# stjude-rust-labs/ngs

Measured on AMD Instinct MI355X. Metric: BAM records/sec (whole node), all qc facets, 150 bp reads, higher is better.
Workload: dtype u8/u32 integer (u64 accumulators)

## Files before the change

ngs_amd/csrc/qual_kernel.hip:

```cpp
#include <hip/hip_runtime.h>

#include <cstdlib>

#include "kernels.h"

namespace ngsq {

typedef unsigned long long u64;

__host__ __device__ constexpr uint32_t qw_rp(uint32_t R) {
    const uint32_t want = R < 12 ? R : 12;
    for (uint32_t rp = R; rp < R + 8; rp++) {
        const uint32_t s = (4 * rp) % 32, d = s < 32 - s ? s : 32 - s;
        if (d >= want) return rp;
    }
    return R;
}
__host__ __device__ constexpr uint32_t qw_cp(uint32_t R) { return (16 * qw_rp(R) + 31) / 32 * 32; }

uint32_t qual_window_lds_bytes(uint32_t R) { return QUAL_BINS * qw_cp(R) * 4; }

template <uint32_t R>
__global__ __launch_bounds__(1024) void k_qual_win(DeviceState st, const uint8_t *__restrict__ qual, uint64_t n_rec,
                                                   uint32_t pitch) {
    NGSQ_FOREGROUND_WAVE();
    constexpr uint32_t RP = qw_rp(R), CP = qw_cp(R), CP4 = CP * 4, RP4 = RP * 4;
    constexpr uint32_t S4 = 4u * RP4;
    constexpr uint32_t magicR = R == 1 ? 0u : (uint32_t)(((1ull << 32) + R - 1) / R);
    extern __shared__ uint32_t s_q[];
    constexpr uint32_t nb = QUAL_BINS * CP;
    for (uint32_t i = threadIdx.x; i < nb; i += blockDim.x) s_q[i] = 0;
    __syncthreads();

    const uint32_t rem = pitch - 16u * (R - 1);
    const uint64_t n_win = n_rec * R;
    const uint64_t per = (n_win + gridDim.x - 1) / gridDim.x;
    const uint64_t lo = min(per * blockIdx.x, n_win), hi = min(lo + per, n_win);
    const uint64_t rec_lo = lo / R;
    const uint32_t tl0 = (uint32_t)(lo - rec_lo * R) + threadIdx.x;
    const uint32_t rl0 = R == 1 ? tl0 : __umulhi(tl0, magicR);
    uint32_t w = tl0 - rl0 * R;
    uint32_t rot = rl0 & 3u;
    constexpr uint32_t STEP_R = 1024 / R, STEP_W = 1024 % R;
    const uint32_t d0 = STEP_R * pitch + 16u * STEP_W, d1 = d0 + pitch - 16u * R;
    const uint8_t *p = qual + (rec_lo + rl0) * (uint64_t)pitch + 16u * w;
    uint32_t bad = 0;
    char *const tab = reinterpret_cast<char *>(s_q);

    auto exact = [&](const uint32_t (&x)[4], uint32_t w_) {
        const uint32_t nvalid = (w_ == R - 1) ? rem : 16u;
        for (uint32_t j = 0; j < nvalid; j++) {
            const uint32_t q = (x[j >> 2] >> (8 * (j & 3))) & 0xFFu;
            if (q <= NGSQ_MAX_SCORE)
                atomicAdd(reinterpret_cast<uint32_t *>(tab + q * CP4 + 4u * w_ + j * RP4), 1u);
            else if (q != 0xFFu)
                bad += 1;
        }
    };
    auto tally = [&](const uint4 &cur, uint32_t w_, uint32_t rot_) {
        const uint32_t ww[4] = {cur.x, cur.y, cur.z, cur.w};
        const uint32_t any = (ww[0] | ww[1] | ww[2] | ww[3]) & 0xC0C0C0C0u;
        if (__builtin_expect(any == 0u, 1)) {
            const uint32_t wbase = 4u * w_;
            uint32_t x[4], bd[4];
            const bool r1 = rot_ & 1u, r2 = rot_ & 2u;
            const uint32_t y0 = r2 ? ww[2] : ww[0], y1 = r2 ? ww[3] : ww[1], y2 = r2 ? ww[0] : ww[2],
                           y3 = r2 ? ww[1] : ww[3];
            x[0] = r1 ? y1 : y0;
            x[1] = r1 ? y0 : y1;
            x[2] = r1 ? y3 : y2;
            x[3] = r1 ? y2 : y3;
            const uint32_t h = r2 ? 2u * S4 : 0u, l = r1 ? S4 : 0u;
            bd[0] = wbase + h + l;
            bd[1] = wbase + h + (S4 - l);
            bd[2] = wbase + (2u * S4 - h) + l;
            bd[3] = wbase + (2u * S4 - h) + (S4 - l);
#pragma unroll
            for (uint32_t d = 0; d < 4; d++) {
#pragma unroll
                for (uint32_t k = 0; k < 4; k++) {
                    const uint32_t q = (x[d] >> (8 * k)) & 0xFFu;
                    atomicAdd(reinterpret_cast<uint32_t *>(tab + (__umul24(q, CP4) + bd[d]) + k * RP4), 1u);
                }
            }
        } else {
            exact(ww, w_);
        }
    };
    auto load = [&](const uint8_t *q) -> uint4 {
        uint4 v;
        __builtin_memcpy(&v, q, 16);
        return v;
    };

    const uint64_t hi_fast = min(hi, n_win - 1);
    uint64_t t = lo + threadIdx.x;
    if (t < hi_fast) {
        uint4 cur = load(p);
        while (t + 1024 < hi_fast) {
            uint32_t w_n = w + STEP_W;
            const bool wrap = w_n >= R;
            w_n = wrap ? w_n - R : w_n;
            p += wrap ? d1 : d0;
            const uint4 nxt = load(p);
            tally(cur, w, rot);
            cur = nxt;
            w = w_n;
            rot = (rot + STEP_R + (wrap ? 1u : 0u)) & 3u;
            t += 1024;
        }
        tally(cur, w, rot);
        t += 1024;
    }
    if (hi == n_win && n_win > 0 && (n_win - 1 - lo) % 1024 == threadIdx.x && n_win - 1 >= lo) {
        uint32_t x[4] = {0, 0, 0, 0};
        const uint64_t off = (n_rec - 1) * (uint64_t)pitch + 16u * (R - 1);
        for (uint32_t k = 0; k < rem; k++) x[k >> 2] |= (uint32_t)qual[off + k] << (8 * (k & 3));
        exact(x, R - 1);
    }
    __syncthreads();
    const uint32_t n_out = pitch * QUAL_BINS;
    for (uint32_t i = threadIdx.x; i < n_out; i += blockDim.x) {
        const uint32_t c = i / QUAL_BINS, q = i - c * QUAL_BINS;
        const uint32_t v = s_q[q * CP + (c & 15u) * RP + (c >> 4)];
        if (v) atomicAdd(&st.counters[st.off_qual + i], (u64)v);
    }
    uint32_t r = bad;
#pragma unroll
    for (int o = 32; o > 0; o >>= 1) r += __shfl_down(r, o, 64);
    if ((threadIdx.x & 63) == 0 && r) atomicAdd(&st.counters[C_ERR + E_BAD_QUAL], (u64)r);
}

__device__ __forceinline__ uint32_t qr_wave_inclusive_sum(uint32_t v) {
    v += (uint32_t)__builtin_amdgcn_update_dpp(0, (int)v, 0x111, 0xF, 0xF, false);
    v += (uint32_t)__builtin_amdgcn_update_dpp(0, (int)v, 0x112, 0xF, 0xF, false);
    v += (uint32_t)__builtin_amdgcn_update_dpp(0, (int)v, 0x114, 0xF, 0xF, false);
    v += (uint32_t)__builtin_amdgcn_update_dpp(0, (int)v, 0x118, 0xF, 0xF, false);
    v += (uint32_t)__builtin_amdgcn_update_dpp(0, (int)v, 0x142, 0xA, 0xF, false);
    v += (uint32_t)__builtin_amdgcn_update_dpp(0, (int)v, 0x143, 0xC, 0xF, false);
    return v;
}
constexpr uint32_t QR_ROWS = 64;
constexpr uint32_t QR_TRASH = QR_ROWS;
constexpr uint32_t QR_FLUSH_EVERY = 63;
__host__ __device__ constexpr uint32_t qr_cp(uint32_t R) { return (8 * qw_rp(R) + 31) / 32 * 32; }
__host__ __device__ constexpr uint32_t qr_table_bytes(uint32_t R) { return (QR_ROWS + 1) * qr_cp(R) * 4; }
__device__ __forceinline__ uint32_t qr_from_lane(uint32_t v, uint32_t src_lane) {
    return (uint32_t)__builtin_amdgcn_ds_bpermute((int)(src_lane << 2), (int)v);
}

template <uint32_t R>
__global__ __launch_bounds__(1024) void k_qual_ragged(DeviceState st, const uint8_t *__restrict__ qual,
                                                      const uint64_t *__restrict__ qual_off, uint64_t n_rec) {
    NGSQ_FOREGROUND_WAVE();
    constexpr uint32_t RP = qw_rp(R), CP = qr_cp(R), CP4 = CP * 4, RP4 = RP * 4;
    constexpr uint32_t S4 = 2u * RP4;
    extern __shared__ uint32_t s_q[];
    constexpr uint32_t nb = (QR_ROWS + 1) * CP;
    for (uint32_t i = threadIdx.x; i < nb; i += blockDim.x) s_q[i] = 0;
    char *const tab = reinterpret_cast<char *>(s_q);
    const uint32_t lane = threadIdx.x & 63u, wave = threadIdx.x >> 6;
    uint8_t *const map = reinterpret_cast<uint8_t *>(s_q + nb) + wave * (64u * R);
    uint4 *const keep_tab = reinterpret_cast<uint4 *>(reinterpret_cast<uint8_t *>(s_q + nb) + 16u * 64u * R);
    if (threadIdx.x <= 16u) {
        uint32_t k[4];
        for (uint32_t d = 0; d < 4; d++) {
            const uint32_t nvd = threadIdx.x > 4u * d ? min(threadIdx.x - 4u * d, 4u) : 0u;
            k[d] = nvd >= 4u ? 0xFFFFFFFFu : (1u << (8u * nvd)) - 1u;
        }
        keep_tab[threadIdx.x] = make_uint4(k[0], k[1], k[2], k[3]);
    }
    __syncthreads();
    const uint64_t per = (n_rec + gridDim.x - 1) / gridDim.x;
    const uint64_t lo = min(per * blockIdx.x, n_rec), hi = min(lo + per, n_rec);
    const uint64_t end_bytes = n_rec ? qual_off[n_rec] : 0;
    uint32_t bad = 0, too_long = 0;
    u64 *const gq = st.counters + st.off_qual;
    const uint32_t n_cyc = min(st.max_read_len, 16u * R);
    auto flush = [&]() {
        __syncthreads();
        for (uint32_t i = threadIdx.x; i < n_cyc * QR_ROWS; i += blockDim.x) {
            const uint32_t c = i / QR_ROWS, q = i - c * QR_ROWS, kb = c & 15u;
            const uint32_t v = (s_q[q * CP + (kb >> 1) * RP + (c >> 4)] >> (16u * (kb & 1u))) & 0xFFFFu;
            if (v) atomicAdd(&gq[(uint64_t)c * QUAL_BINS + q], (u64)v);
        }
        __syncthreads();
        for (uint32_t i = threadIdx.x; i < QR_ROWS * CP; i += blockDim.x) s_q[i] = 0;
        __syncthreads();
    };

    auto load_offs = [&](uint64_t i0, uint64_t &o0, uint64_t &o1) {
        const uint64_t rec = i0 + lane;
        o0 = qual_off[rec < n_rec ? rec : n_rec];
        o1 = qual_off[rec + 1 < n_rec ? rec + 1 : n_rec];
    };
    uint64_t nx_o0 = 0, nx_o1 = 0;
    if (lo + 64ull * wave < hi) load_offs(lo + 64ull * wave, nx_o0, nx_o1);
    const uint64_t n_iter = (hi - lo + 1023) / 1024;
    for (uint64_t it = 0; it < n_iter; it++) {
        if (it && it % QR_FLUSH_EVERY == 0) flush();
        const uint64_t i0 = lo + it * 1024 + 64ull * wave;
        if (i0 >= hi) continue;
        const uint64_t rec = i0 + lane;
        const uint64_t cur_o0 = nx_o0, cur_o1 = nx_o1;
        load_offs(i0 + 64ull * 16, nx_o0, nx_o1);
        uint64_t off = 0;
        uint32_t len = 0;
        if (rec < hi) {
            off = cur_o0;
            const uint64_t l64 = cur_o1 - off;
            len = (uint32_t)min(l64, (uint64_t)st.max_read_len);
            too_long += l64 > st.max_read_len;
        }
        const uint32_t nwin = (len + 15u) >> 4;
        const uint32_t P = qr_wave_inclusive_sum(nwin);
        const uint32_t T = __builtin_amdgcn_readlane(P, 63);
        const uint64_t off0 = ((uint64_t)(uint32_t)__builtin_amdgcn_readfirstlane((int)(off >> 32)) << 32) |
                              (uint32_t)__builtin_amdgcn_readfirstlane((int)(uint32_t)off);
        const uint32_t rel = rec < hi ? (uint32_t)(off - off0) : 0u;
        const uint32_t first_win = P - nwin;
        const uint32_t fw_len = first_win | len << 16;
        for (uint32_t j = 0; __ballot(j < nwin); j++)
            if (j < nwin) map[first_win + j] = (uint8_t)lane;
        __builtin_amdgcn_fence(__ATOMIC_ACQ_REL, "wavefront");
        __builtin_amdgcn_wave_barrier();
        struct Sched {
            uint32_t r, w, nv, sh;
            bool active;
            uint4 v;
        };
        const uint64_t g0 = min(off0, end_bytes - 16);
        const uint32_t delta = (uint32_t)(off0 - g0), lim = (uint32_t)min(end_bytes - 16 - g0, (uint64_t)0xFFFFFFFFu);
        const uint8_t *const gbase = qual + g0;
        auto fetch = [&](uint32_t t0) -> Sched {
            Sched sc;
            const uint32_t t = t0 + lane;
            sc.active = t < T;
            const uint32_t tt = sc.active ? t : (t0 < T ? t0 : 0u);
            sc.r = map[tt];
            const uint32_t fl = qr_from_lane(fw_len, sc.r);
            sc.w = tt - (fl & 0xFFFFu);
            const uint32_t l = fl >> 16;
            sc.nv = sc.w == (l >> 4) ? (l & 15u) : 16u;
            const uint32_t at = qr_from_lane(rel, sc.r) + 16u * sc.w + delta, at_c = min(at, lim);
            sc.sh = at - at_c;
            __builtin_memcpy(&sc.v, gbase + at_c, 16);
            return sc;
        };
        Sched nx{};
        if (T) nx = fetch(0);
        for (uint32_t t0 = 0; t0 < T; t0 += 64) {
            const Sched cu = nx;
            nx = fetch(t0 + 64 < T ? t0 + 64 : t0);
            const bool active = cu.active;
            const uint32_t r = cu.r, w = cu.w, nv = cu.nv;
            if (!active) continue;
            uint32_t ww[4] = {cu.v.x, cu.v.y, cu.v.z, cu.v.w};
            if (__builtin_expect(cu.sh != 0u, 0)) {
                u64 l64 = (u64)ww[1] << 32 | ww[0], h64 = (u64)ww[3] << 32 | ww[2];
                const uint32_t sb = 8u * cu.sh;
                if (sb >= 64u) {
                    l64 = h64 >> (sb - 64u);
                    h64 = 0;
                } else {
                    l64 = l64 >> sb | h64 << (64u - sb);
                    h64 >>= sb;
                }
                ww[0] = (uint32_t)l64, ww[1] = (uint32_t)(l64 >> 32), ww[2] = (uint32_t)h64, ww[3] = (uint32_t)(h64 >> 32);
            }
            const uint4 kp = keep_tab[nv];
            const uint32_t keep[4] = {kp.x, kp.y, kp.z, kp.w};
            const uint32_t any = ((ww[0] & keep[0]) | (ww[1] & keep[1]) | (ww[2] & keep[2]) | (ww[3] & keep[3])) & 0xC0C0C0C0u;
            if (__builtin_expect(any == 0u, 1)) {
                const uint32_t wbase = 4u * w, rot = r & 3u;
                uint32_t x[4], bd[4];
#pragma unroll
                for (uint32_t d = 0; d < 4; d++) ww[d] = (ww[d] & keep[d]) | (~keep[d] & (QR_TRASH * 0x01010101u));
                const bool r1 = rot & 1u, r2 = rot & 2u;
                const uint32_t y0 = r2 ? ww[2] : ww[0], y1 = r2 ? ww[3] : ww[1], y2 = r2 ? ww[0] : ww[2],
                               y3 = r2 ? ww[1] : ww[3];
                x[0] = r1 ? y1 : y0;
                x[1] = r1 ? y0 : y1;
                x[2] = r1 ? y3 : y2;
                x[3] = r1 ? y2 : y3;
                const uint32_t h = r2 ? 2u * S4 : 0u, l = r1 ? S4 : 0u;
                bd[0] = wbase + h + l;
                bd[1] = wbase + h + (S4 - l);
                bd[2] = wbase + (2u * S4 - h) + l;
                bd[3] = wbase + (2u * S4 - h) + (S4 - l);
#pragma unroll
                for (uint32_t d = 0; d < 4; d++) {
#pragma unroll
                    for (uint32_t k = 0; k < 4; k++) {
                        const uint32_t q = (x[d] >> (8 * k)) & 0xFFu;
                        atomicAdd(reinterpret_cast<uint32_t *>(tab + (__umul24(q, CP4) + bd[d]) + (k >> 1) * RP4), 1u << (16u * (k & 1u)));
                    }
                }
            } else {
                for (uint32_t j = 0; j < nv; j++) {
                    const uint32_t q = (ww[j >> 2] >> (8 * (j & 3))) & 0xFFu;
                    if (q < QR_ROWS)
                        atomicAdd(reinterpret_cast<uint32_t *>(tab + q * CP4 + 4u * w + (j >> 1) * RP4), 1u << (16u * (j & 1u)));
                    else if (q <= NGSQ_MAX_SCORE)
                        atomicAdd(&gq[(uint64_t)(16u * w + j) * QUAL_BINS + q], (u64)1);
                    else
                        bad += 1;
                }
            }
        }
        __builtin_amdgcn_fence(__ATOMIC_ACQ_REL, "wavefront");
        __builtin_amdgcn_wave_barrier();
    }
    flush();
    uint32_t r0 = bad, r1 = too_long;
#pragma unroll
    for (int o = 32; o > 0; o >>= 1) {
        r0 += __shfl_down(r0, o, 64);
        r1 += __shfl_down(r1, o, 64);
    }
    if (lane == 0 && r0) atomicAdd(&st.counters[C_ERR + E_BAD_QUAL], (u64)r0);
    if (lane == 0 && r1) atomicAdd(&st.counters[C_ERR + E_READ_TOO_LONG], (u64)r1);
}

template <uint32_t R>
static hipError_t launch_ragged_r(const LaunchInfo &li, const DeviceState &st, const DeviceBatch &b, hipStream_t s) {
    const uint32_t lds = qr_table_bytes(R) + 16u * 64u * R + 17u * 16u;
    static bool attr = false;
    if (!attr) {
        hipError_t e = hipFuncSetAttribute(reinterpret_cast<const void *>(k_qual_ragged<R>),
                                           hipFuncAttributeMaxDynamicSharedMemorySize, (int)lds);
        if (e != hipSuccess) return e;
        attr = true;
    }
    const uint32_t per_cu = lds <= 78 * 1024 ? 2 : 1;
    uint64_t g = (b.n + 1023) / 1024;
    if (g > (uint64_t)li.n_cu * per_cu) g = (uint64_t)li.n_cu * per_cu;
    if (g < 1) g = 1;
    hipLaunchKernelGGL((k_qual_ragged<R>), dim3((uint32_t)g), dim3(1024), lds, s, st, b.qual, b.qual_off, b.n);
    return hipGetLastError();
}

bool qual_ragged_supported(const DeviceState &st, const DeviceBatch &b) {
    return b.qual_off != nullptr && st.max_read_len <= 16 * QUAL_WIN_MAX_R && b.qual_bytes >= 16;
}

hipError_t launch_qual_ragged(const LaunchInfo &li, const DeviceState &st, const DeviceBatch &b, hipStream_t s) {
    const uint32_t R = (st.max_read_len + 15) / 16;
    if (R <= 5) return launch_ragged_r<5>(li, st, b, s);
    if (R <= 10) return launch_ragged_r<10>(li, st, b, s);
    if (R <= 16) return launch_ragged_r<16>(li, st, b, s);
    return launch_ragged_r<20>(li, st, b, s);
}

constexpr uint32_t QP_MAX_R = 16;
constexpr uint32_t QP_LDS_BYTES = 64 * 1024;
typedef __attribute__((address_space(3))) uint32_t lds_u32;

__host__ __device__ constexpr uint32_t qp_threads(uint32_t R) { return R * (1024u / R); }

static __device__ __noinline__ uint32_t qp_exact(u64 *__restrict__ qual_counters, uint32_t x0, uint32_t x1, uint32_t x2,
                                                 uint32_t x3, uint32_t w, uint32_t nvalid) {
    const uint32_t x[4] = {x0, x1, x2, x3};
    uint32_t bad = 0;
    for (uint32_t j = 0; j < nvalid; j++) {
        const uint32_t q = (x[j >> 2] >> (8 * (j & 3))) & 0xFFu;
        if (q < 64u) {
            lds_u32 *cell = reinterpret_cast<lds_u32 *>((j >> 2) * 16384u + q * 256u + w * 16u + (j & 3u) * 4u);
            __hip_atomic_fetch_add(cell, 1u, __ATOMIC_RELAXED, __HIP_MEMORY_SCOPE_WORKGROUP);
        } else if (q <= NGSQ_MAX_SCORE) {
            atomicAdd(&qual_counters[(uint64_t)(16u * w + j) * QUAL_BINS + q], (u64)1);
        } else if (q != 0xFFu) {
            bad += 1;
        }
    }
    return bad;
}

template <uint32_t R, uint32_t D>
__global__ __launch_bounds__(1024) void k_qual_perm(DeviceState st, const uint8_t *__restrict__ qual, uint64_t n_rec,
                                                    uint32_t pitch) {
    NGSQ_FOREGROUND_WAVE();
    static_assert(R >= 1 && R <= QP_MAX_R, "window index must fit the low byte of a table address");
    constexpr uint32_t T = qp_threads(R), RPB = T / R;
    constexpr uint32_t magicR = R == 1 ? 0u : (uint32_t)(((1ull << 32) + R - 1) / R);
    extern __shared__ uint32_t s_q[];
    if (reinterpret_cast<uintptr_t>((lds_u32 *)s_q) != 0) __builtin_trap();
    for (uint32_t i = threadIdx.x; i < QP_LDS_BYTES / 4; i += T) s_q[i] = 0;
    __syncthreads();

    const uint32_t rem = pitch - 16u * (R - 1);
    const uint32_t r0 = R == 1 ? threadIdx.x : __umulhi(threadIdx.x, magicR);
    const uint32_t w = threadIdx.x - r0 * R;
    const uint64_t per = (n_rec + gridDim.x - 1) / gridDim.x;
    const uint64_t lo = min(per * blockIdx.x, n_rec), hi = min(lo + per, n_rec);
    const uint64_t step = (uint64_t)RPB * pitch;
    const uint8_t *pf = qual + (lo + r0) * (uint64_t)pitch + 16u * w;
    u64 *const qc = st.counters + st.off_qual;

    uint32_t sel[4];
#pragma unroll
    for (uint32_t k = 0; k < 4; k++) {
        const uint32_t kk = (k + r0) & 3u;
        sel[k] = 0x0C0C0000u | ((4u + kk) << 8) | kk;
    }
    const uint32_t cvec = w * 0x10101010u + 0x0C080400u;

    uint32_t n_it = lo + r0 < hi ? (uint32_t)((hi - lo - r0 + RPB - 1) / RPB) : 0u;
    const bool owns_last = n_it > 0 && w == R - 1 && lo + r0 + (uint64_t)(n_it - 1) * RPB == n_rec - 1;
    if (owns_last) n_it -= 1;

    uint32_t bad = 0;
    auto tally = [&](const uint4 &v) {
        const uint32_t any = (v.x | v.y | v.z | v.w) & 0xC0C0C0C0u;
        if (__builtin_expect(any == 0u, 1)) {
            const uint32_t x[4] = {v.x, v.y, v.z, v.w};
#pragma unroll
            for (uint32_t d = 0; d < 4; d++) {
#pragma unroll
                for (uint32_t k = 0; k < 4; k++) {
                    const uint32_t a = __builtin_amdgcn_perm(x[d], cvec, sel[k]);
                    lds_u32 *cell = reinterpret_cast<lds_u32 *>(a) + d * 4096u;
                    __hip_atomic_fetch_add(cell, 1u, __ATOMIC_RELAXED, __HIP_MEMORY_SCOPE_WORKGROUP);
                }
            }
        } else {
            bad += qp_exact(qc, v.x, v.y, v.z, v.w, w, w == R - 1 ? rem : 16u);
        }
    };
    auto load = [&]() -> uint4 {
        uint4 v;
        __builtin_memcpy(&v, pf, 16);
        pf += step;
        return v;
    };

    constexpr uint32_t NB = D + 1;
    uint4 buf[NB];
#pragma unroll
    for (uint32_t j = 0; j < D; j++)
        if (j < n_it) buf[j] = load();
    uint32_t done = 0;
    for (; done + NB + D <= n_it; done += NB) {
#pragma unroll
        for (uint32_t j = 0; j < NB; j++) {
            buf[(j + D) % NB] = load();
            tally(buf[j]);
        }
    }
#pragma unroll
    for (uint32_t j = 0; j < NB + D; j++) {
        if (done + j < n_it) {
            if (done + j + D < n_it) buf[(j + D) % NB] = load();
            tally(buf[j % NB]);
        }
    }

    if (owns_last) {
        uint32_t x[4] = {0, 0, 0, 0};
        const uint64_t off = (n_rec - 1) * (uint64_t)pitch + 16u * (R - 1);
        for (uint32_t k = 0; k < rem; k++) x[k >> 2] |= (uint32_t)qual[off + k] << (8 * (k & 3));
        bad += qp_exact(qc, x[0], x[1], x[2], x[3], R - 1, rem);
    }
    __syncthreads();
    for (uint32_t i = threadIdx.x; i < QP_LDS_BYTES / 4; i += T) {
        const uint32_t v = s_q[i];
        if (v) {
            const uint32_t d = i >> 12, q = (i >> 6) & 63u, c = ((i >> 2) & 15u) * 16u + d * 4u + (i & 3u);
            if (c < pitch) atomicAdd(&qc[(uint64_t)c * QUAL_BINS + q], (u64)v);
        }
    }
    uint32_t r = bad;
#pragma unroll
    for (int o = 32; o > 0; o >>= 1) r += __shfl_down(r, o, 64);
    if ((threadIdx.x & 63) == 0 && r) atomicAdd(&st.counters[C_ERR + E_BAD_QUAL], (u64)r);
}

template <uint32_t R, uint32_t D>
static hipError_t launch_perm(const LaunchInfo &li, const DeviceState &st, const DeviceBatch &b, hipStream_t s) {
    static bool attr = false;
    if (!attr) {
        hipError_t e = hipFuncSetAttribute(reinterpret_cast<const void *>(k_qual_perm<R, D>),
                                           hipFuncAttributeMaxDynamicSharedMemorySize, (int)QP_LDS_BYTES);
        if (e != hipSuccess) return e;
        attr = true;
    }
    constexpr uint32_t RPB = qp_threads(R) / R;
    uint64_t g = (b.n + RPB - 1) / RPB;
    if (g > (uint64_t)li.n_cu * 2) g = (uint64_t)li.n_cu * 2;
    if (g < 1) g = 1;
    hipLaunchKernelGGL((k_qual_perm<R, D>), dim3((uint32_t)g), dim3(qp_threads(R)), QP_LDS_BYTES, s, st, b.qual, b.n,
                       b.qual_stride);
    return hipGetLastError();
}

template <uint32_t D>
static hipError_t dispatch_perm(uint32_t R, const LaunchInfo &li, const DeviceState &st, const DeviceBatch &b,
                                hipStream_t s) {
    switch (R) {
#define CASE(r) \
    case r: return launch_perm<r, D>(li, st, b, s);
        CASE(1) CASE(2) CASE(3) CASE(4) CASE(5) CASE(6) CASE(7) CASE(8) CASE(9) CASE(10) CASE(11) CASE(12) CASE(13)
        CASE(14) CASE(15) CASE(16)
#undef CASE
    default: return hipErrorInvalidValue;
    }
}

template <uint32_t R>
static hipError_t launch_r(const LaunchInfo &li, const DeviceState &st, const DeviceBatch &b, hipStream_t s) {
    const uint32_t lds = qual_window_lds_bytes(R);
    static bool attr = false;
    if (!attr) {
        hipError_t e = hipFuncSetAttribute(reinterpret_cast<const void *>(k_qual_win<R>),
                                           hipFuncAttributeMaxDynamicSharedMemorySize, (int)lds);
        if (e != hipSuccess) return e;
        attr = true;
    }
    const uint32_t per_cu = lds <= 78 * 1024 ? 2 : 1;
    uint64_t g = (b.n * R + 1023) / 1024;
    if (g > (uint64_t)li.n_cu * per_cu) g = (uint64_t)li.n_cu * per_cu;
    if (g < 1) g = 1;
    hipLaunchKernelGGL((k_qual_win<R>), dim3((uint32_t)g), dim3(1024), lds, s, st, b.qual, b.n, b.qual_stride);
    return hipGetLastError();
}

static hipError_t dispatch(uint32_t R, const LaunchInfo &li, const DeviceState &st, const DeviceBatch &b,
                           hipStream_t s) {
    switch (R) {
#define CASE(r) \
    case r: return launch_r<r>(li, st, b, s);
        CASE(1) CASE(2) CASE(3) CASE(4) CASE(5) CASE(6) CASE(7) CASE(8) CASE(9) CASE(10) CASE(11) CASE(12) CASE(13)
        CASE(14) CASE(15) CASE(16) CASE(17) CASE(18) CASE(19) CASE(20)
#undef CASE
    default: return hipErrorInvalidValue;
    }
}

bool qual_window_supported(const DeviceState &st, const DeviceBatch &b) {
    return !b.qual_off && b.qual_stride >= 1 && b.qual_stride <= st.max_read_len && b.qual_stride <= 16 * QUAL_WIN_MAX_R;
}

hipError_t launch_qual_window(const LaunchInfo &li, const DeviceState &st, const DeviceBatch &b, hipStream_t s) {
    const uint32_t R = (b.qual_stride + 15) / 16;
    if (R <= QP_MAX_R) return dispatch_perm<2>(R, li, st, b, s);
    return dispatch(R, li, st, b, s);
}

}
```

Baseline: 19.49 billion.

## Treat quality buffer as a flat aligned 16-byte stream with periodic column mapping

The permuted-LDS quality histogram kernel now walks the whole padded quality buffer as one contiguous array of aligned 16-byte words, not as per-record windows of 16*R bytes. Each thread precomputes byte-order and column-offset vectors for its fixed column phase, using the period of pitch in 16-byte words, so the hot loop stays a perm plus an LDS atomic per byte. The goal is fully coalesced aligned loads with no wasted lanes on the partial last window of each record (150 bp gives 10 windows with a 6-byte tail), and one non-templated kernel. In exchange the setup is more complex, the first and last words need unaligned edge handling, and the thread-to-column mapping depends on pitch periodicity, which limits how work can be split across blocks.

```diff
diff --git a/ngs_amd/csrc/qual_kernel.hip b/ngs_amd/csrc/qual_kernel.hip
--- a/ngs_amd/csrc/qual_kernel.hip
+++ b/ngs_amd/csrc/qual_kernel.hip
@@ -352,89 +352,127 @@
     return launch_ragged_r<20>(li, st, b, s);
 }
 
-constexpr uint32_t QP_MAX_R = 16;
+constexpr uint32_t QP_MAX_PITCH = 256;
 constexpr uint32_t QP_LDS_BYTES = 64 * 1024;
 typedef __attribute__((address_space(3))) uint32_t lds_u32;
 
-__host__ __device__ constexpr uint32_t qp_threads(uint32_t R) { return R * (1024u / R); }
+static uint32_t qp_period(uint32_t pitch) {
+    const uint32_t low = pitch & (0u - pitch);
+    return pitch / (low < 16u ? low : 16u);
+}
+constexpr uint32_t QP_THREADS = 1024;
 
 static __device__ __noinline__ uint32_t qp_exact(u64 *__restrict__ qual_counters, uint32_t x0, uint32_t x1, uint32_t x2,
-                                                 uint32_t x3, uint32_t w, uint32_t nvalid) {
+                                                 uint32_t x3, uint32_t c0, uint32_t pitch, uint32_t j_lo, uint32_t j_hi) {
     const uint32_t x[4] = {x0, x1, x2, x3};
-    uint32_t bad = 0;
-    for (uint32_t j = 0; j < nvalid; j++) {
+    uint32_t bad = 0, c = (c0 + j_lo) % pitch;
+    for (uint32_t j = j_lo; j < j_hi; j++) {
         const uint32_t q = (x[j >> 2] >> (8 * (j & 3))) & 0xFFu;
         if (q < 64u) {
-            lds_u32 *cell = reinterpret_cast<lds_u32 *>((j >> 2) * 16384u + q * 256u + w * 16u + (j & 3u) * 4u);
+            lds_u32 *cell = reinterpret_cast<lds_u32 *>(((c >> 2) & 3u) * 16384u + q * 256u + (c >> 4) * 16u + (c & 3u) * 4u);
             __hip_atomic_fetch_add(cell, 1u, __ATOMIC_RELAXED, __HIP_MEMORY_SCOPE_WORKGROUP);
         } else if (q <= NGSQ_MAX_SCORE) {
-            atomicAdd(&qual_counters[(uint64_t)(16u * w + j) * QUAL_BINS + q], (u64)1);
+            atomicAdd(&qual_counters[(uint64_t)c * QUAL_BINS + q], (u64)1);
         } else if (q != 0xFFu) {
             bad += 1;
         }
+        c = c + 1 == pitch ? 0u : c + 1;
     }
     return bad;
 }
 
-template <uint32_t R, uint32_t D>
-__global__ __launch_bounds__(1024) void k_qual_perm(DeviceState st, const uint8_t *__restrict__ qual, uint64_t n_rec,
-                                                    uint32_t pitch) {
+__global__ __launch_bounds__(1024) void k_qual_perm(DeviceState st, const uint8_t *__restrict__ qual, uint64_t n_bytes,
+                                                    uint32_t pitch, uint32_t W) {
     NGSQ_FOREGROUND_WAVE();
-    static_assert(R >= 1 && R <= QP_MAX_R, "window index must fit the low byte of a table address");
-    constexpr uint32_t T = qp_threads(R), RPB = T / R;
-    constexpr uint32_t magicR = R == 1 ? 0u : (uint32_t)(((1ull << 32) + R - 1) / R);
     extern __shared__ uint32_t s_q[];
     if (reinterpret_cast<uintptr_t>((lds_u32 *)s_q) != 0) __builtin_trap();
-    for (uint32_t i = threadIdx.x; i < QP_LDS_BYTES / 4; i += T) s_q[i] = 0;
+    constexpr uint32_t T = QP_THREADS;
+    const uint32_t t = threadIdx.x;
+    for (uint32_t i = t; i < QP_LDS_BYTES / 4; i += T) s_q[i] = 0;
     __syncthreads();
 
-    const uint32_t rem = pitch - 16u * (R - 1);
-    const uint32_t r0 = R == 1 ? threadIdx.x : __umulhi(threadIdx.x, magicR);
-    const uint32_t w = threadIdx.x - r0 * R;
-    const uint64_t per = (n_rec + gridDim.x - 1) / gridDim.x;
-    const uint64_t lo = min(per * blockIdx.x, n_rec), hi = min(lo + per, n_rec);
-    const uint64_t step = (uint64_t)RPB * pitch;
-    const uint8_t *pf = qual + (lo + r0) * (uint64_t)pitch + 16u * w;
+    const uint32_t m = (uint32_t)(reinterpret_cast<uintptr_t>(qual) & 15u);
+    const uint8_t *const stream = qual - m;
+    const uint64_t n_str = m + n_bytes;
+    const uint64_t n_win = n_bytes ? (n_str + 15) / 16 : 0;
+    const uint32_t w_low = W & (0u - W), n_slots = W / (w_low < 64u ? w_low : 64u);
+    const uint64_t stride = 64ull * n_slots;
+    const uint32_t g = blockIdx.x * (T / 64) + (t >> 6), n_runs = gridDim.x * (T / 64) / n_slots;
+    const uint32_t pos = 64u * (g % n_slots) + (t & 63u);
+    const uint64_t n_sr = (n_win + stride - 1) / stride, per = (n_sr + n_runs - 1) / n_runs;
+    const uint64_t run = g / n_slots, lo_sr = min(per * run, n_sr), hi_sr = run < n_runs ? min(lo_sr + per, n_sr) : lo_sr;
+    const uint64_t first = lo_sr * stride + pos, hi = min(hi_sr * stride, n_win);
+    const uint4 *pf = reinterpret_cast<const uint4 *>(stream) + first;
     u64 *const qc = st.counters + st.off_qual;
 
-    uint32_t sel[4];
-#pragma unroll
-    for (uint32_t k = 0; k < 4; k++) {
-        const uint32_t kk = (k + r0) & 3u;
-        sel[k] = 0x0C0C0000u | ((4u + kk) << 8) | kk;
-    }
-    const uint32_t cvec = w * 0x10101010u + 0x0C080400u;
-
-    uint32_t n_it = lo + r0 < hi ? (uint32_t)((hi - lo - r0 + RPB - 1) / RPB) : 0u;
-    const bool owns_last = n_it > 0 && w == R - 1 && lo + r0 + (uint64_t)(n_it - 1) * RPB == n_rec - 1;
+    const uint32_t c0 = (16u * pos + 16u * pitch - m) % pitch;
+    uint32_t ord[4], addv[4], lowv[4];
+    {
+        uint32_t c = c0, row = ((16u * (pos % W) + 16u * W - m) % (16u * W)) / pitch + pos / W;
+#pragma unroll
+        for (uint32_t d = 0; d < 4; d++) {
+            uint32_t low = 0, taken = 0, late = 0;
+            ord[d] = addv[d] = 0;
+#pragma unroll
+            for (uint32_t b = 0; b < 4; b++) {
+                low |= ((c & 0xF0u) | ((c & 3u) << 2)) << (8 * b);
+                addv[d] |= ((c >> 2) & 3u) << (8 * b + 6);
+                const uint32_t k = (c - row) & 3u;
+                if (taken >> k & 1u) {
+                    late |= 1u << b;
+                } else {
+                    taken |= 1u << k;
+                    ord[d] |= b << (8 * k);
+                }
+                c += 1;
+                if (c == pitch) c = 0, row += 1;
+            }
+#pragma unroll
+            for (uint32_t b = 0; b < 4; b++) {
+                if (late >> b & 1u) {
+                    const uint32_t k = (uint32_t)__builtin_ctz(~taken);
+                    taken |= 1u << k;
+                    ord[d] |= b << (8 * k);
+                }
+            }
+            lowv[d] = __builtin_amdgcn_perm(low, low, ord[d]);
+        }
+    }
+
+    uint32_t n_it = first < hi ? (uint32_t)((hi - first + stride - 1) / stride) : 0u;
+    const bool owns_last = n_it > 0 && first + (uint64_t)(n_it - 1) * stride == n_win - 1;
+    const bool owns_first = m != 0 && n_it > 0 && first == 0;
     if (owns_last) n_it -= 1;
+    if (owns_first && n_it > 0) {
+        pf += stride;
+        n_it -= 1;
+    }
 
     uint32_t bad = 0;
     auto tally = [&](const uint4 &v) {
         const uint32_t any = (v.x | v.y | v.z | v.w) & 0xC0C0C0C0u;
         if (__builtin_expect(any == 0u, 1)) {
-            const uint32_t x[4] = {v.x, v.y, v.z, v.w};
+            const uint32_t y[4] = {v.x + addv[0], v.y + addv[1], v.z + addv[2], v.w + addv[3]};
 #pragma unroll
             for (uint32_t d = 0; d < 4; d++) {
+                const uint32_t x = __builtin_amdgcn_perm(y[d], y[d], ord[d]);
 #pragma unroll
                 for (uint32_t k = 0; k < 4; k++) {
-                    const uint32_t a = __builtin_amdgcn_perm(x[d], cvec, sel[k]);
-                    lds_u32 *cell = reinterpret_cast<lds_u32 *>(a) + d * 4096u;
-                    __hip_atomic_fetch_add(cell, 1u, __ATOMIC_RELAXED, __HIP_MEMORY_SCOPE_WORKGROUP);
+                    const uint32_t a = __builtin_amdgcn_perm(x, lowv[d], 0x0C0C0400u + 0x0101u * k);
+                    __hip_atomic_fetch_add(reinterpret_cast<lds_u32 *>(a), 1u, __ATOMIC_RELAXED, __HIP_MEMORY_SCOPE_WORKGROUP);
                 }
             }
         } else {
-            bad += qp_exact(qc, v.x, v.y, v.z, v.w, w, w == R - 1 ? rem : 16u);
+            bad += qp_exact(qc, v.x, v.y, v.z, v.w, c0, pitch, 0u, 16u);
         }
     };
     auto load = [&]() -> uint4 {
-        uint4 v;
-        __builtin_memcpy(&v, pf, 16);
-        pf += step;
+        const uint4 v = *pf;
+        pf += stride;
         return v;
     };
 
-    constexpr uint32_t NB = D + 1;
+    constexpr uint32_t D = 2, NB = D + 1;
     uint4 buf[NB];
 #pragma unroll
     for (uint32_t j = 0; j < D; j++)
@@ -455,55 +493,43 @@
         }
     }
 
-    if (owns_last) {
+    auto edge = [&](uint64_t g, uint32_t j_lo, uint32_t j_hi) {
         uint32_t x[4] = {0, 0, 0, 0};
-        const uint64_t off = (n_rec - 1) * (uint64_t)pitch + 16u * (R - 1);
-        for (uint32_t k = 0; k < rem; k++) x[k >> 2] |= (uint32_t)qual[off + k] << (8 * (k & 3));
-        bad += qp_exact(qc, x[0], x[1], x[2], x[3], R - 1, rem);
-    }
+        for (uint32_t j = j_lo; j < j_hi; j++) x[j >> 2] |= (uint32_t)stream[16 * g + j] << (8 * (j & 3));
+        bad += qp_exact(qc, x[0], x[1], x[2], x[3], c0, pitch, j_lo, j_hi);
+    };
+    if (owns_last) edge(n_win - 1, n_win == 1 ? m : 0u, (uint32_t)(n_str - 16 * (n_win - 1)));
+    if (owns_first && n_win > 1) edge(0, m, 16u);
     __syncthreads();
-    for (uint32_t i = threadIdx.x; i < QP_LDS_BYTES / 4; i += T) {
+    for (uint32_t i = t; i < QP_LDS_BYTES / 4; i += T) {
         const uint32_t v = s_q[i];
         if (v) {
             const uint32_t d = i >> 12, q = (i >> 6) & 63u, c = ((i >> 2) & 15u) * 16u + d * 4u + (i & 3u);
-            if (c < pitch) atomicAdd(&qc[(uint64_t)c * QUAL_BINS + q], (u64)v);
+            atomicAdd(&qc[(uint64_t)c * QUAL_BINS + q], (u64)v);
         }
     }
     uint32_t r = bad;
 #pragma unroll
     for (int o = 32; o > 0; o >>= 1) r += __shfl_down(r, o, 64);
-    if ((threadIdx.x & 63) == 0 && r) atomicAdd(&st.counters[C_ERR + E_BAD_QUAL], (u64)r);
-}
-
-template <uint32_t R, uint32_t D>
+    if ((t & 63) == 0 && r) atomicAdd(&st.counters[C_ERR + E_BAD_QUAL], (u64)r);
+}
+
 static hipError_t launch_perm(const LaunchInfo &li, const DeviceState &st, const DeviceBatch &b, hipStream_t s) {
     static bool attr = false;
     if (!attr) {
-        hipError_t e = hipFuncSetAttribute(reinterpret_cast<const void *>(k_qual_perm<R, D>),
+        hipError_t e = hipFuncSetAttribute(reinterpret_cast<const void *>(k_qual_perm),
                                            hipFuncAttributeMaxDynamicSharedMemorySize, (int)QP_LDS_BYTES);
         if (e != hipSuccess) return e;
         attr = true;
     }
-    constexpr uint32_t RPB = qp_threads(R) / R;
-    uint64_t g = (b.n + RPB - 1) / RPB;
+    const uint32_t W = qp_period(b.qual_stride), T = QP_THREADS;
+    const uint64_t n_bytes = b.n * (uint64_t)b.qual_stride;
+    const uint64_t n_win = (n_bytes + (reinterpret_cast<uintptr_t>(b.qual) & 15u) + 15) / 16;
+    uint64_t g = (n_win + T - 1) / T;
     if (g > (uint64_t)li.n_cu * 2) g = (uint64_t)li.n_cu * 2;
-    if (g < 1) g = 1;
-    hipLaunchKernelGGL((k_qual_perm<R, D>), dim3((uint32_t)g), dim3(qp_threads(R)), QP_LDS_BYTES, s, st, b.qual, b.n,
-                       b.qual_stride);
+    if (g < (W + 15) / 16) g = (W + 15) / 16;
+    hipLaunchKernelGGL((k_qual_perm), dim3((uint32_t)g), dim3(T), QP_LDS_BYTES, s, st, b.qual, n_bytes, b.qual_stride, W);
     return hipGetLastError();
-}
-
-template <uint32_t D>
-static hipError_t dispatch_perm(uint32_t R, const LaunchInfo &li, const DeviceState &st, const DeviceBatch &b,
-                                hipStream_t s) {
-    switch (R) {
-#define CASE(r) \
-    case r: return launch_perm<r, D>(li, st, b, s);
-        CASE(1) CASE(2) CASE(3) CASE(4) CASE(5) CASE(6) CASE(7) CASE(8) CASE(9) CASE(10) CASE(11) CASE(12) CASE(13)
-        CASE(14) CASE(15) CASE(16)
-#undef CASE
-    default: return hipErrorInvalidValue;
-    }
 }
 
 template <uint32_t R>
@@ -541,9 +567,8 @@
 }
 
 hipError_t launch_qual_window(const LaunchInfo &li, const DeviceState &st, const DeviceBatch &b, hipStream_t s) {
-    const uint32_t R = (b.qual_stride + 15) / 16;
-    if (R <= QP_MAX_R) return dispatch_perm<2>(R, li, st, b, s);
-    return dispatch(R, li, st, b, s);
-}
-
-}
+    if (b.qual_stride <= QP_MAX_PITCH) return launch_perm(li, st, b, s);
+    return dispatch((b.qual_stride + 15) / 16, li, st, b, s);
+}
+
+}
```

Result: faster. 19.80 billion, median of 6 (+1.6%).
